# NicholasMilef/UUO-Mocap

Measured on AMD Instinct MI355X. Metric: mocap frames/sec fitted (300-frame seq, 50 markers), higher is better.
Workload: dtype f32

## Files before the change

uuo_mocap_amd/_lib.py:

```python
from __future__ import annotations

import ctypes
import os
import re
from ctypes import POINTER, c_char_p, c_float, c_int, c_int32, c_void_p

_HERE = os.path.dirname(os.path.abspath(__file__))
LIB_PATH = os.path.join(_HERE, "libuuo_hip.so")
HEADER_PATH = os.path.join(os.path.dirname(_HERE), "include", "uuo_hip.h")

UUO_STAGE_CHAMFER, UUO_STAGE_MARKER, UUO_STAGE_PART = 0, 1, 2


ABI_VERSION = 3


class UuoProblem(ctypes.Structure):
    _fields_ = [
        ("stage", c_int32), ("F", c_int32), ("M", c_int32),
        ("d_markers", c_void_p), ("d_o_pose", c_void_p), ("d_o_betas", c_void_p), ("d_root", c_void_p),
        ("d_assign", c_void_p), ("d_subset", c_void_p), ("n_subset", c_int32),
        ("w_data", c_float), ("w_pose", c_float), ("w_betas", c_float), ("marker_distance", c_float),
        ("pose_cache_id", ctypes.c_uint64),
        ("w_soft", c_float), ("soft_tau", c_float),
# ... 12 lines not shown
    _fields_ = [
        ("n_iter", c_int32), ("n_eval", c_int32), ("first_loss", c_float), ("final_loss", c_float),
        ("stop_reason", c_int32), ("device_ms", c_float),
    ]


class UuoReprojectionProblem(ctypes.Structure):
    _fields_ = [
        ("F", c_int32), ("M", c_int32), ("V", c_int32), ("J", c_int32),
        ("d_markers", c_void_p), ("d_joints0", c_void_p), ("d_verts0", c_void_p), ("d_kp_target", c_void_p),
        ("d_mask", c_void_p), ("focal", c_float * 2), ("center", c_float * 2),
        ("w_reprojection", c_float), ("w_chamfer", c_float),
    ]


EVAL_CALLBACK = ctypes.CFUNCTYPE(None, c_void_p, c_int, c_float, c_void_p)
GATHER_FN = ctypes.CFUNCTYPE(c_int, c_void_p, POINTER(ctypes.c_double), c_int, POINTER(ctypes.c_double))


class UuoShared(ctypes.Structure):
    _fields_ = [("gather", GATHER_FN), ("user", c_void_p), ("rank", c_int32), ("world", c_int32)]


_SIGNATURES = {
    "uuo_last_error": (c_char_p, []),
    "uuo_abi_version": (c_int, []),
    "uuo_model_create": (c_int, [c_void_p] * 7 + [c_int, POINTER(c_void_p)]),
    "uuo_model_destroy": (c_int, [c_void_p]),
    "uuo_model_num_verts": (c_int, [c_void_p]),
    "uuo_smpl_forward": (c_int, [c_void_p, c_void_p, c_int, c_void_p, c_void_p, c_int, c_void_p, c_void_p,
                                 c_void_p, c_void_p]),
    "uuo_smpl_backward": (c_int, [c_void_p, c_void_p, c_int, c_void_p, c_void_p, c_int, c_void_p, c_void_p, c_void_p,
                                  c_void_p, c_void_p, c_void_p, c_void_p, c_void_p, c_void_p]),
    "uuo_nn_argmin": (c_int, [c_void_p, c_int, c_int, c_int, c_void_p, c_void_p, c_void_p, c_int, c_void_p,
                              c_void_p, c_void_p]),
    "uuo_rigid_distance_std": (c_int, [c_void_p, c_int, c_int, c_void_p, c_void_p]),
    "uuo_assign_mean_argmin": (c_int, [c_void_p, c_int, c_int, c_int, c_void_p, c_void_p, c_void_p, c_void_p,
                                       c_void_p]),
    "uuo_soft_nn_forward": (c_int, [c_void_p, c_int, c_int, c_int, c_void_p, c_void_p, c_float, c_void_p, c_void_p,
                                    c_void_p, c_void_p]),
    "uuo_soft_nn_backward": (c_int, [c_void_p, c_int, c_int, c_int, c_void_p, c_void_p, c_float, c_void_p, c_void_p,
                                     c_void_p, c_void_p, c_void_p]),
    "uuo_copy_to_host": (c_int, [c_void_p, c_void_p, c_void_p, c_int]),
    "uuo_mesh_closest_points": (c_int, [c_void_p, c_int, c_int, c_int, c_int, c_void_p, c_void_p, c_void_p, c_void_p,
                                        c_void_p, c_void_p, c_void_p]),
    "uuo_fit_create": (c_int, [c_void_p, c_int, c_int, POINTER(c_void_p)]),
    "uuo_fit_destroy": (c_int, [c_void_p]),
    "uuo_problem_num_params": (c_int, [POINTER(UuoProblem)]),
    "uuo_closure_eval": (c_int, [c_void_p, c_void_p, POINTER(UuoProblem), c_void_p, c_void_p, c_void_p, c_void_p]),
    "uuo_lbfgs_solve": (c_int, [c_void_p, c_void_p, POINTER(UuoProblem), c_void_p, POINTER(UuoLbfgsOptions),
                                POINTER(UuoLbfgsStats), c_void_p, c_void_p]),
    "uuo_lbfgs_solve_shared": (c_int, [c_void_p, c_void_p, POINTER(UuoProblem), c_void_p, POINTER(UuoLbfgsOptions),
                                       POINTER(UuoLbfgsStats), POINTER(UuoShared), c_void_p, c_void_p]),
    "uuo_time_closure": (c_int, [c_void_p, c_void_p, POINTER(UuoProblem), c_void_p, c_int, c_int,
                                 POINTER(c_float)]),
    "uuo_lbfgs_minimize": (c_int, [c_void_p, c_int, c_void_p, POINTER(UuoLbfgsOptions), POINTER(UuoLbfgsStats), c_void_p,
                                   c_void_p, c_void_p, c_void_p]),
    "uuo_reprojection_create": (c_int, [POINTER(UuoReprojectionProblem), POINTER(c_void_p)]),
    "uuo_reprojection_destroy": (c_int, [c_void_p]),
    "uuo_reprojection_num_params": (c_int, [POINTER(UuoReprojectionProblem)]),
    "uuo_reprojection_eval": (c_int, [c_void_p, c_void_p, c_void_p, c_void_p, c_void_p, c_void_p, c_void_p]),
    "uuo_reprojection_solve": (c_int, [c_void_p, c_void_p, c_void_p, POINTER(UuoLbfgsOptions), POINTER(UuoLbfgsStats),
                                       c_void_p, c_void_p, c_void_p, c_void_p]),
    "uuo_set_wait_policy": (c_int, [c_int, c_int]),
    "uuo_mailbox_open": (c_int, [c_char_p, c_int32, c_int32, ctypes.c_double, POINTER(c_void_p)]),
    "uuo_mailbox_close": (c_int, [c_void_p]),
    "uuo_mailbox_gather": (c_int, [c_void_p, c_void_p, c_int, c_void_p]),
    "uuo_mailbox_stats": (c_int, [c_void_p, POINTER(ctypes.c_ulonglong), POINTER(ctypes.c_ulonglong)]),
    "uuo_copy_device": (c_int, [c_void_p, c_void_p, c_void_p, ctypes.c_size_t]),
    "uuo_batch_create": (c_int, [c_void_p, c_int, c_int, c_int, c_int, POINTER(c_void_p)]),
    "uuo_batch_destroy": (c_int, [c_void_p]),
    "uuo_batch_solve": (c_int, [c_void_p, c_void_p, POINTER(UuoProblem), POINTER(c_void_p), c_int,
                                POINTER(UuoLbfgsOptions), POINTER(UuoLbfgsStats)]),
    "uuo_batch_part_scores": (c_int, [c_void_p, c_void_p, POINTER(UuoProblem), POINTER(c_void_p), c_int,
                                      POINTER(c_float)]),
}
LIB_DEBUG_PATH = os.path.join(_HERE, "libuuo_hip_debug.so")
_DEBUG_SIGNATURES = {
    "uuo_lbfgs_selftest": (c_int, [c_void_p, c_int, c_int, c_void_p, POINTER(UuoLbfgsOptions),
                                   POINTER(UuoLbfgsStats), c_void_p, c_void_p]),
    "uuo_debug_fit_buffers": (c_int, [c_void_p, c_void_p, c_void_p]),
    "uuo_debug_nn_flags": (c_int, [c_void_p, c_void_p]),
    "uuo_debug_skin16_check": (c_int, [c_void_p, c_int]),
    "uuo_debug_small_coeffs": (c_int, [c_int, c_int, c_int, c_void_p]),
    "uuo_debug_time_small": (c_int, [c_int, c_int, c_int, POINTER(c_float)]),
    "uuo_debug_index_map": (c_int, [c_int, c_int, c_int, c_void_p]),
    "uuo_debug_staging_script": (c_int, [c_void_p, c_int, ctypes.c_longlong, c_void_p]),
}

CLOSURE_FN = ctypes.CFUNCTYPE(c_int, c_void_p, c_void_p, c_void_p, c_void_p, c_void_p)

_lib = None
_lib_debug = None


def header_symbols():
    text = open(HEADER_PATH).read()
    text = re.sub(r"/\*.*?\*/", "", text, flags=re.S)
    names = re.findall(r"\b(uuo_[a-z0-9_]+)\s*\(", text)
    return sorted(set(n for n in names if n != "uuo_eval_callback_t"))


def load():
    global _lib
    if _lib is not None:
        return _lib
    if not os.path.isfile(LIB_PATH):
        raise RuntimeError(
            "libuuo_hip.so is missing (%s): run `python __graft_entry__.py` to build the HIP extension. "
            "There is no CPU fallback for the fitted path." % LIB_PATH)
    lib = ctypes.CDLL(LIB_PATH)
    for name in header_symbols():
        if not hasattr(lib, name):
            raise RuntimeError("libuuo_hip.so does not export %s declared in include/uuo_hip.h" % name)
    for name, (res, args) in _SIGNATURES.items():
        fn = getattr(lib, name)
        fn.restype = res
        fn.argtypes = args
    if lib.uuo_abi_version() != ABI_VERSION:
        raise RuntimeError("libuuo_hip.so has ABI version %d, this package binds version %d: rebuild it "
                           "(python __graft_entry__.py)" % (lib.uuo_abi_version(), ABI_VERSION))
    _lib = lib
    return lib


def load_debug():
    global _lib_debug
    if _lib_debug is not None:
        return _lib_debug
    if not os.path.isfile(LIB_DEBUG_PATH):
        raise RuntimeError("libuuo_hip_debug.so is missing (%s): run `python __graft_entry__.py`" % LIB_DEBUG_PATH)
    lib = ctypes.CDLL(LIB_DEBUG_PATH)
    for name, (res, args) in list(_SIGNATURES.items()) + list(_DEBUG_SIGNATURES.items()):
        fn = getattr(lib, name)
        fn.restype = res
        fn.argtypes = args
    _lib_debug = lib
    return lib


def check(rc: int, what: str = ""):
    if rc != 0:
        msg = load().uuo_last_error()
        raise RuntimeError("%s failed (%d): %s" % (what or "libuuo_hip call", rc, msg.decode() if msg else ""))
```

uuo_mocap_amd/csrc/smpl_kernels.hip:

```cpp
#include <cstdlib>

#include "frame_math.h"


__device__ __forceinline__ void pose_prep_body(const UuoPoseSrc& src, const UuoTree* __restrict__ tree, int F,
                                               float* __restrict__ pfaT, float* __restrict__ A,
                                               float* __restrict__ jposed, float* __restrict__ frames,
                                               const float* __restrict__ ST = nullptr, const int* __restrict__ Wi = nullptr,
                                               const float* __restrict__ Ww = nullptr, int V = 0,
                                               const int32_t* __restrict__ subset = nullptr, int ns = 0,
                                               float* __restrict__ sb_out = nullptr, _Float16* __restrict__ pfa16 = nullptr) {
  __builtin_amdgcn_s_setprio(3);
  __shared__ FrameLds L;
  const int f = blockIdx.x;
  const int l = threadIdx.x;
  frame_forward(src, tree, f, L);
  if (frames) {
    constexpr int NW = sizeof(FrameLds) / 4;
    const float* src_l = reinterpret_cast<const float*>(&L);
    for (int i = l; i < NW; i += 64) frames[(size_t)f * NW + i] = src_l[i];
  }
  const int ft = f / UUO_FT, i = f % UUO_FT;
  float* tile = pfaT + (size_t)ft * UUO_KP * UUO_FT;
  _Float16* tile16 = pfa16 ? pfa16 + (size_t)ft * UUO_KP * UUO_FT * 2 : nullptr;
// ... 566 lines not shown
    ra[0] = pa[0];
#pragma unroll
    for (int g = 0; g < SKIN_GROUPS; ++g) {
      const int st = g % SK2_RING;
      const float4 av = ra[g & 1];
      const int part = g % 3;
      const int k_aread = (g < 12 && part == 2) ? 11 : 10;
#pragma unroll
      for (int k = 0; k < 12; ++k) {
        const int ks = k / 3, c = k - 3 * ks;
        const float a = (ks == 0) ? av.x : (ks == 1) ? av.y : (ks == 2) ? av.z : av.w;
        if (VAR & 4) {
          asm volatile("" ::"v"(a), "v"(rbuf[c][st][ks]));
        } else if (c == 0) {
          acc0 = __builtin_amdgcn_mfma_f32_16x16x4f32(a, rbuf[0][st][ks], acc0, 0, 0, 0);
        } else if (c == 1) {
          acc1 = __builtin_amdgcn_mfma_f32_16x16x4f32(a, rbuf[1][st][ks], acc1, 0, 0, 0);
        } else {
          acc2 = __builtin_amdgcn_mfma_f32_16x16x4f32(a, rbuf[2][st][ks], acc2, 0, 0, 0);
        }
        if (!(VAR & 1) && g < 12) sk2_slice<BBOX, VPOUT>(g, k, E, ww, q0, q1, q2, sTb, sTrb, v12, n24, rv, rb, rvp);
        if (k == k_aread && g + 1 < SKIN_GROUPS) ra[(g + 1) & 1] = pa[(g + 1) * 64];
        if (g == 2 && k == 11) {
          const int t_n = __builtin_amdgcn_readfirstlane(claimed);
          more = t_n < tb1;
          t_nxt = more ? t_n : t_cur;
          SK2_DECODE(nxt, t_nxt);
          pbn = (unsigned)nxt.u * (SKIN_GROUPS * 1024u);
        }
        if (g == 11 && k == 10) {
          wi = __builtin_bit_cast(int4, __builtin_amdgcn_raw_buffer_load_b128(rwi, j16, cur.u * 256, 0));
          ww = __builtin_bit_cast(float4, __builtin_amdgcn_raw_buffer_load_b128(rww, j16, cur.u * 256, 0));
          tn0 = __builtin_bit_cast(float, __builtin_amdgcn_raw_buffer_load_b32(rvt, j4, nxt.u * 64, 0));
          tn1 = __builtin_bit_cast(float, __builtin_amdgcn_raw_buffer_load_b32(rvt, j4, VP * 4 + nxt.u * 64, 0));
          tn2 = __builtin_bit_cast(float, __builtin_amdgcn_raw_buffer_load_b32(rvt, j4, VP * 8 + nxt.u * 64, 0));
        }
        __builtin_amdgcn_sched_barrier(0);
      }
      if (!(VAR & 2)) {
        const unsigned ub = (g + SK2_RING < SKIN_GROUPS) ? pb : pbn;
        const int gg = (g + SK2_RING) % SKIN_GROUPS;
        rbuf[0][st] = SK2_LDB(0, ub, gg);
        rbuf[1][st] = SK2_LDB(1, ub, gg);
        rbuf[2][st] = SK2_LDB(2, ub, gg);
      }
      __builtin_amdgcn_sched_barrier(0);
    }
    if (VAR & 8) {
      typedef unsigned u32x2 __attribute__((ext_vector_type(2)));
      const unsigned long long c = __builtin_readcyclecounter();
      const u32x2 cv = {(unsigned)c, (unsigned)(c >> 32)};
      const unsigned so = (unsigned)(((blockIdx.x * SKIN_WAVES + wave) * 16 + 2 + (nunits_done < 8 ? nunits_done : 7)) * 8);
      __builtin_amdgcn_raw_buffer_store_b64(cv, rst, so | (lane == 0 ? 0u : 0x80000000u), 0, 0);
    }
    ++nunits_done;
    q0 = acc0; q1 = acc1; q2 = acc2;
    prv = cur; cur = nxt; pb = pbn; t_cur = t_nxt;
    sk2_unit_addresses(E, prv, wi, kq, j, V, v12, n24);
  }
#undef SK2_LDB
#undef SK2_DECODE
#pragma unroll
  for (int g = 0; g < 12; ++g) {
#pragma unroll
    for (int k = 0; k < 12; ++k) sk2_slice<BBOX, VPOUT>(g, k, E, ww, q0, q1, q2, sTb, sTrb, v12, n24, rv, rb, rvp);
  }
  if ((VAR & 8) && lane == 0) {
    unsigned long long* o = g_sk2_stamps + (size_t)(blockIdx.x * SKIN_WAVES + wave) * 16;
    o[0] = stamp0; o[1] = stamp1;
    o[10] = __builtin_readcyclecounter();
    o[11] = (unsigned long long)nunits_done;
    o[12] = stampS;
  }
}

typedef _Float16 f16x8 __attribute__((ext_vector_type(8)));
#define SK3_STEPS (SKIN_GROUPS / 2)
#define SK3_NMFMA (SK3_STEPS * 9)
#define SK3_NSLICE 144

#ifndef SK3_WAVES
#define SK3_WAVES 4
#endif
#ifndef SK3_LDS_PAD
#define SK3_LDS_PAD 44288
#endif
template <bool BBOX>
__global__ __launch_bounds__(SK3_WAVES * 64) __attribute__((amdgpu_waves_per_eu(1, 1))) void k_skin3(
    const float4* __restrict__ P16v, const float* __restrict__ vt3, const int* __restrict__ Wi, const float* __restrict__ Ww,
    const float4* __restrict__ pfa16, const float* __restrict__ A, const float* __restrict__ trans, float* __restrict__ verts,
    float* __restrict__ bbox, int F, int V, int VP, int nFT, float inv_scale) {
  __shared__ float4 sA[2 * UUO_KP * UUO_FT / 4];
  __shared__ f32x4 sT[2 * UUO_FT * UUO_NUM_JOINTS * 3];
  __shared__ float4 sTr[2 * UUO_FT];
  __shared__ int sQ[64];
  const int tid = threadIdx.x;
  const int wave = __builtin_amdgcn_readfirstlane(tid >> 6), lane = tid & 63;
  const int j = lane & 15, kq = lane >> 4;
  const int nunits = VP / 16;
  const int nur = (V + 15) / 16;
  const int xcd = blockIdx.x & 7, pos = blockIdx.x >> 3;
  const int ntot = nFT * nur;
  const int xlo = (int)(((unsigned)ntot * (unsigned)xcd) >> 3), xhi = (int)(((unsigned)ntot * (unsigned)(xcd + 1)) >> 3);
  const int tb0 = xlo + (((xhi - xlo) * pos) >> SK2_NPOS_LOG2), tb1 = xlo + (((xhi - xlo) * (pos + 1)) >> SK2_NPOS_LOG2);
  if (tb1 <= tb0) return;
  int xa = 0;
  while (xa < 7 && nFT * (((xa + 1) * nur) >> 3) <= tb0) ++xa;
  const int ua0 = (xa * nur) >> 3, ub0 = ((xa + 1) * nur) >> 3;
  const int nua = ub0 - ua0;
  const int Sa = nFT * ua0, Sb = nFT * ub0;
  const int ftA = (tb0 - Sa) / nua;
  const int g1 = Sa + ftA * nua;
  const int g2 = (g1 + nua < Sb) ? g1 + nua : Sb;
  const int ftB = (tb1 - 1 < Sb) ? ftA + 1 : 0;
  const int nslots = (tb1 > g2) ? 2 : 1;

  const __amdgpu_buffer_rsrc_t rv = __builtin_amdgcn_make_buffer_rsrc(verts, 0, F * V * 12, 0x00020000);
  const __amdgpu_buffer_rsrc_t rb = __builtin_amdgcn_make_buffer_rsrc(bbox, 0, BBOX ? F * nur * 24 : 0, 0x00020000);
  const unsigned cplane = (unsigned)nunits * SKIN_GROUPS * 1024u;
  const __amdgpu_buffer_rsrc_t rp =
      __builtin_amdgcn_make_buffer_rsrc(const_cast<float4*>(P16v), 0, (int)(3u * cplane), 0x00020000);
  const __amdgpu_buffer_rsrc_t rwi = __builtin_amdgcn_make_buffer_rsrc(const_cast<int*>(Wi), 0, VP * 16, 0x00020000);
  const __amdgpu_buffer_rsrc_t rww = __builtin_amdgcn_make_buffer_rsrc(const_cast<float*>(Ww), 0, VP * 16, 0x00020000);
  const __amdgpu_buffer_rsrc_t rvt = __builtin_amdgcn_make_buffer_rsrc(const_cast<float*>(vt3), 0, VP * 12, 0x00020000);
  const unsigned lane16 = lane * 16, j16 = j * 16, j4 = j * 4;
#define SK3_LDB(c, ubase, g) \
  __builtin_bit_cast(f32x4, __builtin_amdgcn_raw_buffer_load_b128(rp, lane16, (ubase) + (c)*cplane + (g)*1024u, 0))
#define SK3_DECODE(U, t_)                                                        \
  {                                                                              \
    const bool s1_ = (t_) < g2;                                                  \
    const int base_ = s1_ ? g1 : ((t_) < Sb ? g2 : Sb);                          \
    (U).u = (((t_) < Sb) ? ua0 : ub0) + (t_)-base_;                              \
    (U).i0 = (s1_ ? ftA : ftB) * UUO_FT;                                         \
    (U).slot = s1_ ? 0 : 1;                                                      \
  }

  constexpr int NA = UUO_KP * UUO_FT / 4, NT = UUO_FT * UUO_NUM_JOINTS * 3;
  constexpr int PER = (2 * (NA + NT) + SK3_WAVES * 64 - 1) / (SK3_WAVES * 64);
  float4 tmp[PER];
  float4 trv = make_float4(0.f, 0.f, 0.f, 0.f);
  {
    const float4* gA0 = pfa16 + (size_t)ftA * NA;
    const float4* gA1 = pfa16 + (size_t)ftB * NA;
    const float4* gT0 = reinterpret_cast<const float4*>(A + (size_t)ftA * UUO_FT * UUO_NUM_JOINTS * 12);
    const float4* gT1 = reinterpret_cast<const float4*>(A + (size_t)ftB * UUO_FT * UUO_NUM_JOINTS * 12);
#pragma unroll
    for (int r = 0; r < PER; ++r) {
      const int i = tid + r * SK3_WAVES * 64;
      tmp[r] = make_float4(0.f, 0.f, 0.f, 0.f);
      if (i < NA) tmp[r] = gA0[i];
      else if (i < 2 * NA) { if (nslots > 1) tmp[r] = gA1[i - NA]; }
      else if (i < 2 * NA + NT) tmp[r] = gT0[i - 2 * NA];
      else if (i < 2 * NA + 2 * NT) { if (nslots > 1) tmp[r] = gT1[i - 2 * NA - NT]; }
    }
    if (tid < 2 * UUO_FT) {
      const int f = ((tid < UUO_FT) ? ftA : ftB) * UUO_FT + (tid & (UUO_FT - 1));
      if (trans && f < F && (tid < UUO_FT || nslots > 1))
        trv = make_float4(trans[(size_t)f * 3], trans[(size_t)f * 3 + 1], trans[(size_t)f * 3 + 2], 0.f);
    }
  }

  int t_cur = tb0 + wave;
  const bool active = t_cur < tb1;
  if (!active) t_cur = tb0;
  Sk2Unit cur, prv, nxt;
  SK3_DECODE(cur, t_cur);
  prv.u = cur.u; prv.i0 = F; prv.slot = 0;
  nxt = cur;
  unsigned pb = (unsigned)cur.u * (SKIN_GROUPS * 1024u);
  f32x4 rbuf[3][SK2_RING];
#pragma unroll
  for (int s = 0; s < SK2_RING; ++s) {
    rbuf[0][s] = SK3_LDB(0, pb, s);
    rbuf[1][s] = SK3_LDB(1, pb, s);
    rbuf[2][s] = SK3_LDB(2, pb, s);
  }

  if (tid < 64) sQ[tid] = (tid == 0) ? tb0 + SK3_WAVES : 0;
#pragma unroll
  for (int r = 0; r < PER; ++r) {
    const int i = tid + r * SK3_WAVES * 64;
    if (i < 2 * NA) sA[i] = tmp[r];
    else if (i < 2 * (NA + NT)) sT[i - 2 * NA] = __builtin_bit_cast(f32x4, tmp[r]);
  }
  if (tid < 2 * UUO_FT) sTr[tid] = trv;
  __syncthreads();
  if (!active) return;

  int4 wi = make_int4(0, 0, 0, 0);
  float4 ww = make_float4(0.f, 0.f, 0.f, 0.f);
  f32x4 q0 = {0.f, 0.f, 0.f, 0.f}, q1 = q0, q2 = q0;
  Sk2Epi E;
  const char* sTb = reinterpret_cast<const char*>(sT);
  const char* sTrb = reinterpret_cast<const char*>(sTr);
  const unsigned v12 = (unsigned)V * 12u, n24 = (unsigned)nur * 24u;
  sk2_unit_addresses(E, prv, wi, kq, j, V, v12, n24);
  bool more = true;

  while (more) {
    const int claimed = __hip_atomic_fetch_add(&sQ[lane], lane == 0 ? 1 : 0, __ATOMIC_RELAXED, __HIP_MEMORY_SCOPE_WORKGROUP);
    unsigned pbn = pb;
    int t_nxt = t_cur;
    const float tn0 = __builtin_bit_cast(float, __builtin_amdgcn_raw_buffer_load_b32(rvt, j4, cur.u * 64, 0));
    const float tn1 = __builtin_bit_cast(float, __builtin_amdgcn_raw_buffer_load_b32(rvt, j4, VP * 4 + cur.u * 64, 0));
    const float tn2 = __builtin_bit_cast(float, __builtin_amdgcn_raw_buffer_load_b32(rvt, j4, VP * 8 + cur.u * 64, 0));
    const int4 wi_n = __builtin_bit_cast(int4, __builtin_amdgcn_raw_buffer_load_b128(rwi, j16, cur.u * 256, 0));
    const float4 ww_n = __builtin_bit_cast(float4, __builtin_amdgcn_raw_buffer_load_b128(rww, j16, cur.u * 256, 0));
    const float4* pa = sA + cur.slot * (UUO_KP * UUO_FT / 4) + lane;
    f32x4 am0 = {0.f, 0.f, 0.f, 0.f}, am1 = am0, am2 = am0;
    f32x4 as0 = am0, as1 = am0, as2 = am0;
    float4 ah[2], al[2];
    ah[0] = pa[0];
    al[0] = pa[64];
#ifdef SK3_NO_MFMA
#define SK3_MFMA(acc, a_, b_) asm volatile("" : "+v"(acc) : "v"(a_), "v"(b_))
#else
#define SK3_MFMA(acc, a_, b_) asm volatile("v_mfma_f32_16x16x32_f16 %0, %1, %2, %0" : "+v"(acc) : "v"(a_), "v"(b_))
#endif
#define SK3_STEP(ST)                                                         \
    {                                                                        \
      constexpr int st = ST;                                                 \
      constexpr int rh = (2 * st) % SK2_RING, rl = (2 * st + 1) % SK2_RING; \
      const f16x8 a_hi = __builtin_bit_cast(f16x8, ah[st & 1]), a_lo = __builtin_bit_cast(f16x8, al[st & 1]); \
_Pragma("unroll") \
      for (int q = 0; q < 9; ++q) { \
        const int term = q / 3, c = q - 3 * term; \
        const f16x8 b_hi = __builtin_bit_cast(f16x8, rbuf[c][rh]), b_lo = __builtin_bit_cast(f16x8, rbuf[c][rl]); \
        const f16x8 ax = (term == 2) ? a_lo : a_hi, bx = (term == 1) ? b_lo : b_hi; \
        if (term == 0) { \
          if (c == 0) SK3_MFMA(am0, ax, bx); \
          else if (c == 1) SK3_MFMA(am1, ax, bx); \
          else SK3_MFMA(am2, ax, bx); \
        } else { \
          if (c == 0) SK3_MFMA(as0, ax, bx); \
          else if (c == 1) SK3_MFMA(as1, ax, bx); \
          else SK3_MFMA(as2, ax, bx); \
        } \
        const int mslot = st * 9 + q; \
        const int n0 = (mslot * SK3_NSLICE) / SK3_NMFMA, n1 = ((mslot + 1) * SK3_NSLICE) / SK3_NMFMA; \
_Pragma("unroll") \
        for (int i = 0; i < 3; ++i) { \
          const int n = n0 + i; \
          if (n < n1) sk2_slice<BBOX, false, true>(n / 12, n % 12, E, ww, q0, q1, q2, sTb, sTrb, v12, n24, rv, rb, rv); \
        } \
        if (q == 5 && st + 1 < SK3_STEPS) { \
          ah[(st + 1) & 1] = pa[(2 * (st + 1)) * 64]; \
          al[(st + 1) & 1] = pa[(2 * (st + 1) + 1) * 64]; \
        } \
        if (st == 2 && q == 4) { \
          const int t_n = __builtin_amdgcn_readfirstlane(claimed); \
          more = t_n < tb1; \
          t_nxt = more ? t_n : t_cur; \
          SK3_DECODE(nxt, t_nxt); \
          pbn = (unsigned)nxt.u * (SKIN_GROUPS * 1024u); \
        } \
        __builtin_amdgcn_sched_barrier(0); \
      } \
      { \
        constexpr int gh = 2 * st + SK2_RING, gl = 2 * st + 1 + SK2_RING; \
        const unsigned ubh = (gh < SKIN_GROUPS) ? pb : pbn, ubl = (gl < SKIN_GROUPS) ? pb : pbn; \
        rbuf[0][rh] = SK3_LDB(0, ubh, gh % SKIN_GROUPS); \
        rbuf[1][rh] = SK3_LDB(1, ubh, gh % SKIN_GROUPS); \
        rbuf[2][rh] = SK3_LDB(2, ubh, gh % SKIN_GROUPS); \
        rbuf[0][rl] = SK3_LDB(0, ubl, gl % SKIN_GROUPS); \
        rbuf[1][rl] = SK3_LDB(1, ubl, gl % SKIN_GROUPS); \
        rbuf[2][rl] = SK3_LDB(2, ubl, gl % SKIN_GROUPS); \
      } \
      __builtin_amdgcn_sched_barrier(0); \
    }
    SK3_STEP(0) SK3_STEP(1) SK3_STEP(2) SK3_STEP(3) SK3_STEP(4) SK3_STEP(5) SK3_STEP(6)
#undef SK3_STEP
#undef SK3_MFMA
    asm volatile("s_nop 7\n\ts_nop 3");
    __builtin_amdgcn_sched_barrier(0);
    q0 = (am0 + as0) * inv_scale + tn0;
    q1 = (am1 + as1) * inv_scale + tn1;
    q2 = (am2 + as2) * inv_scale + tn2;
    wi = wi_n;
    ww = ww_n;
    prv = cur; cur = nxt; pb = pbn; t_cur = t_nxt;
    sk2_unit_addresses(E, prv, wi, kq, j, V, v12, n24);
  }
#undef SK3_LDB
#undef SK3_DECODE
#pragma unroll
  for (int g = 0; g < 12; ++g) {
#pragma unroll
    for (int k = 0; k < 12; ++k) sk2_slice<BBOX, false, true>(g, k, E, ww, q0, q1, q2, sTb, sTrb, v12, n24, rv, rb, rv);
  }
}

static bool sk2_fits(int nFT, int nur, int npos) {
  if (nur < 8) return false;
  const int ntot = nFT * nur;
  for (int x = 0; x < 8; ++x) {
    const int xlo = (int)(((long)ntot * x) >> 3), xhi = (int)(((long)ntot * (x + 1)) >> 3);
    for (int pos = 0; pos < npos; ++pos) {
      const int tb0 = xlo + (((xhi - xlo) * pos) >> SK2_NPOS_LOG2), tb1 = xlo + (((xhi - xlo) * (pos + 1)) >> SK2_NPOS_LOG2);
      if (tb1 <= tb0) continue;
      int xa = 0;
      while (xa < 7 && nFT * (((xa + 1) * nur) >> 3) <= tb0) ++xa;
      const int ua0 = (xa * nur) >> 3, ub0 = ((xa + 1) * nur) >> 3, nua = ub0 - ua0;
      const int Sa = nFT * ua0, Sb = nFT * ub0;
      const int ftA = (tb0 - Sa) / nua;
      const int g1 = Sa + ftA * nua;
      const int g2 = (g1 + nua < Sb) ? g1 + nua : Sb;
      const bool seg2 = tb1 > g2 && g2 < Sb;
      const bool seg3 = tb1 > Sb;
      if (seg2 && seg3) return false;
      if (seg2 && tb1 > g2 + nua) return false;
      if (seg3 && (xa >= 7 || tb1 - Sb > (((xa + 2) * nur) >> 3) - ub0)) return false;
    }
  }
  return true;
}

static int uuo_launch_skin_v1(const uuo_model* m, hipStream_t s, int F, const float* pfaT, const float* A,
                              const float* trans, float* verts, float* bbox);

struct SkinCallArgs {
  UuoGridHdr h;
  const uuo_model* m;
  int F;
  const float* pfaT;
  const float* A;
  const float* trans;
  float* verts;
  float* bbox;
  const void* pfa16;
};

int uuo_launch_skin(const uuo_model* m, hipStream_t s, int F, const float* pfaT, const float* A, const float* trans,
                    float* verts, float* bbox, float* vp_out) {
  UUO_REQUIRE(!vp_out || (bbox && !uuo_recorder), "uuo_launch_skin: v_posed output goes with the unit boxes, outside lock-step batches");
  {
    SkinCallArgs c{{1, 1}, m, F, pfaT, A, trans, verts, bbox, nullptr};
    if (uuo_record(UUO_OP_SKIN, 1, 1, c)) return 0;
  }
  static const int force_v1 = UUO_ENV_INT("UUO_SKIN_V1", 0);
  const int nur = (m->V + 15) / 16;
  const int npos = 1 << SK2_NPOS_LOG2;
  if (force_v1 || (size_t)SK2_MAX_FT * UUO_FT * m->V * 12 >= 0x7FFFFFF0u) {
    UUO_REQUIRE(!vp_out, "uuo_launch_skin: v_posed output needs the k_skin2 path");
    return uuo_launch_skin_v1(m, s, F, pfaT, A, trans, verts, bbox);
  }
  const int nFT_all = (F + UUO_FT - 1) / UUO_FT;
  for (int ft0 = 0; ft0 < nFT_all; ft0 += SK2_MAX_FT) {
    const int nFT = (nFT_all - ft0 < SK2_MAX_FT) ? nFT_all - ft0 : SK2_MAX_FT;
    const int f0 = ft0 * UUO_FT;
    const int Fl = (F - f0 < nFT * UUO_FT) ? F - f0 : nFT * UUO_FT;
    if (!sk2_fits(nFT, nur, npos)) {
      UUO_REQUIRE(!vp_out, "uuo_launch_skin: v_posed output needs the k_skin2 path");
      return uuo_launch_skin_v1(m, s, F, pfaT, A, trans, verts, bbox);
    }
    const float* pf = pfaT + (size_t)ft0 * UUO_KP * UUO_FT;
    const float* pA = A + (size_t)f0 * UUO_NUM_JOINTS * 12;
    const float* pt = trans ? trans + (size_t)f0 * 3 : nullptr;
    float* pv = verts + (size_t)f0 * m->V * 3;
    static const int var2 = UUO_ENV_INT("UUO_SK2_VAR", 0);
#define SK2_LAUNCH(BB, VAR)                                                                             \
  hipLaunchKernelGGL((k_skin2<BB, VAR>), dim3(8 * npos), dim3(SKIN_WAVES * 64), 0, s,                   \
                     reinterpret_cast<const float4*>(m->P3), m->vt3, m->Wi, m->Ww, pf, pA, pt, pv,      \
                     (BB) ? bbox + (size_t)f0 * nur * 6 : (float*)nullptr, Fl, m->V, m->VP, nFT, (float*)nullptr)
    if (!bbox) SK2_LAUNCH(false, 0);
    else if (vp_out)
      hipLaunchKernelGGL((k_skin2<true, 0, true>), dim3(8 * npos), dim3(SKIN_WAVES * 64), 0, s,
                         reinterpret_cast<const float4*>(m->P3), m->vt3, m->Wi, m->Ww, pf, pA, pt, pv,
                         bbox + (size_t)f0 * nur * 6, Fl, m->V, m->VP, nFT, vp_out + (size_t)f0 * m->V * 3);
#ifdef UUO_DEBUG_HOOKS
    else if (var2 == 1) SK2_LAUNCH(true, 1);
    else if (var2 == 2) SK2_LAUNCH(true, 2);
    else if (var2 == 4) SK2_LAUNCH(true, 4);
    else if (var2 == 3) SK2_LAUNCH(true, 3);
    else if (var2 == 5) SK2_LAUNCH(true, 5);
    else if (var2 == 6) SK2_LAUNCH(true, 6);
    else if (var2 == 7) SK2_LAUNCH(true, 7);
    else if (var2 == 16) SK2_LAUNCH(false, 0);
    else if (var2 == 8) SK2_LAUNCH(true, 8);
    else if (var2 == 9) SK2_LAUNCH(true, 9);
    else if (var2 == 10) SK2_LAUNCH(true, 10);
    else if (var2 == 11) SK2_LAUNCH(true, 11);
    else if (var2 == 12) SK2_LAUNCH(true, 12);
    else if (var2 == 24) SK2_LAUNCH(false, 8);
#endif
    else SK2_LAUNCH(true, 0);
    (void)var2;
#undef SK2_LAUNCH
  }
  UUO_HIP_CHECK(hipGetLastError());
  return 0;
}

#ifdef UUO_DEBUG_HOOKS
extern "C" int uuo_debug_skin_stamps(unsigned long long* h_out) {
  UUO_HIP_CHECK(hipMemcpyFromSymbol(h_out, HIP_SYMBOL(g_sk2_stamps), sizeof(unsigned long long) * 2048 * 16));
  return 0;
}
#endif

int uuo_launch_skin16(const uuo_model* m, hipStream_t s, int F, const void* pfa16, const float* A, const float* trans, float* verts,
                      float* bbox) {
  UUO_REQUIRE(m->P16 && pfa16 && bbox, "uuo_launch_skin16: needs the fp16 tables and the unit boxes");
  static const hipError_t lds_attr =
      hipFuncSetAttribute(reinterpret_cast<const void*>(&k_skin3<true>), hipFuncAttributeMaxDynamicSharedMemorySize, SK3_LDS_PAD);
  UUO_HIP_CHECK(lds_attr);
  const int nur = (m->V + 15) / 16;
  const int npos = 1 << SK2_NPOS_LOG2;
  if ((size_t)SK2_MAX_FT * UUO_FT * m->V * 12 >= 0x7FFFFFF0u) return -22;
  const int nFT_all = (F + UUO_FT - 1) / UUO_FT;
  for (int ft0 = 0; ft0 < nFT_all; ft0 += SK2_MAX_FT) {
    const int nFT = (nFT_all - ft0 < SK2_MAX_FT) ? nFT_all - ft0 : SK2_MAX_FT;
    if (!sk2_fits(nFT, nur, npos)) return -22;
  }
  {
    SkinCallArgs c{{1, 1}, m, F, nullptr, A, trans, verts, bbox, pfa16};
    if (uuo_record(UUO_OP_SKIN, 1, 1, c)) return 0;
  }
  for (int ft0 = 0; ft0 < nFT_all; ft0 += SK2_MAX_FT) {
    const int nFT = (nFT_all - ft0 < SK2_MAX_FT) ? nFT_all - ft0 : SK2_MAX_FT;
    const int f0 = ft0 * UUO_FT;
    const int Fl = (F - f0 < nFT * UUO_FT) ? F - f0 : nFT * UUO_FT;
    hipLaunchKernelGGL((k_skin3<true>), dim3(8 * npos), dim3(SK3_WAVES * 64), SK3_LDS_PAD, s, reinterpret_cast<const float4*>(m->P16), m->vt3,
                       m->Wi, m->Ww, reinterpret_cast<const float4*>(pfa16) + (size_t)ft0 * (UUO_KP * UUO_FT / 4),
                       A + (size_t)f0 * UUO_NUM_JOINTS * 12, trans ? trans + (size_t)f0 * 3 : (const float*)nullptr,
                       verts + (size_t)f0 * m->V * 3, bbox + (size_t)f0 * nur * 6, Fl, m->V, m->VP, nFT, m->skin16_inv);
  }
  UUO_HIP_CHECK(hipGetLastError());
  return 0;
}

static int uuo_launch_skin_v1(const uuo_model* m, hipStream_t s, int F, const float* pfaT, const float* A,
                              const float* trans, float* verts, float* bbox) {
  const int nFT = (F + UUO_FT - 1) / UUO_FT;
  const int nunits = m->VP / 16;
  static const int slots = UUO_ENV_INT("UUO_SKIN_SLOTS", 256);
  int nVB = slots / nFT;
  const int maxVB = (nunits + SKIN_WAVES - 1) / SKIN_WAVES;
  if (nVB > maxVB) nVB = maxVB;
  if (nVB < 1) nVB = 1;
  const int nblocks = nFT * nVB;
  static const int variant = UUO_ENV_INT("UUO_SKIN_VARIANT", 0);
#define SKIN_LAUNCH(VAR)                                                                                     \
  hipLaunchKernelGGL((k_skin<VAR>), dim3(nblocks), dim3(SKIN_WAVES * 64), 0, s, m->P3, m->vt3, m->Wi, m->Ww, \
                     pfaT, A, trans, verts, bbox, F, m->V, m->VP, nFT, nVB, nblocks)
#ifdef UUO_DEBUG_HOOKS
  if (variant == 1) SKIN_LAUNCH(1);
  else if (variant == 2) SKIN_LAUNCH(2);
  else if (variant == 3) SKIN_LAUNCH(3);
  else if (variant == 4) SKIN_LAUNCH(4);
  else if (variant == 5) SKIN_LAUNCH(5);
  else
#endif
    SKIN_LAUNCH(0);
  (void)variant;
#undef SKIN_LAUNCH
  UUO_HIP_CHECK(hipGetLastError());
  return 0;
}

#define SKC_FB 10
__device__ __forceinline__ void skin_cached_body(int F, int V, int ns, const int32_t* __restrict__ subset,
                                                 const float* __restrict__ C, const float* __restrict__ ST,
                                                 const int* __restrict__ Wi, const float* __restrict__ Ww,
                                                 const float* __restrict__ A, const float* __restrict__ betas,
                                                 const float* __restrict__ trans, float* __restrict__ verts,
                                                 float* __restrict__ bbox) {
  __shared__ float sA[SKC_FB * UUO_NUM_JOINTS * 12];
  __shared__ float sTr[SKC_FB * 3];
  const int f0 = blockIdx.y * SKC_FB, nf = min(SKC_FB, F - f0);
  for (int i = threadIdx.x; i < nf * UUO_NUM_JOINTS * 12; i += 256) sA[i] = A[(size_t)f0 * UUO_NUM_JOINTS * 12 + i];
  if (threadIdx.x < nf * 3) sTr[threadIdx.x] = trans ? trans[(size_t)f0 * 3 + threadIdx.x] : 0.f;
  __syncthreads();
  const int i = blockIdx.x * 256 + threadIdx.x;
  const bool compact = bbox != nullptr;
  if (!compact && i >= ns) return;
  if (compact && (i & ~15) >= ns) return;
  const bool mine = i < ns;
  const int ic = mine ? i : ns - 1;
  const int v = subset ? subset[ic] : ic;
  if ((unsigned)v >= (unsigned)V) {
    if (!compact) return;
  }
  const int vs = ((unsigned)v < (unsigned)V) ? v : 0;
  float sb[3] = {0.f, 0.f, 0.f};
#pragma unroll
  for (int c = 0; c < 3; ++c)
#pragma unroll
    for (int l = 0; l < 10; ++l) sb[c] = fmaf(ST[(size_t)vs * 30 + c * 10 + l], betas[l], sb[c]);
  const int4 wi = *reinterpret_cast<const int4*>(Wi + (size_t)vs * 4);
  const float4 ww = *reinterpret_cast<const float4*>(Ww + (size_t)vs * 4);
  const int wj[4] = {wi.x, wi.y, wi.z, wi.w};
  const float wv[4] = {ww.x, ww.y, ww.z, ww.w};
  const int nuc = (ns + 15) >> 4;
  float cx[SKC_FB], cy[SKC_FB], cz[SKC_FB];
#pragma unroll
  for (int q = 0; q < SKC_FB; ++q) {
    const float* pc = C + ((size_t)(f0 + (q < nf ? q : nf - 1)) * V + vs) * 3;
    cx[q] = pc[0]; cy[q] = pc[1]; cz[q] = pc[2];
  }
#pragma unroll
  for (int q = 0; q < SKC_FB; ++q) {
    if (q >= nf) continue;
    const float px = cx[q] + sb[0], py = cy[q] + sb[1], pz = cz[q] + sb[2];
    float T[12];
#pragma unroll
    for (int e = 0; e < 12; ++e) T[e] = 0.f;
#pragma unroll
    for (int n = 0; n < 4; ++n) {
      const float* a = sA + (q * UUO_NUM_JOINTS + (wj[n] < 0 ? 0 : wj[n])) * 12;
      const float w = (wj[n] < 0) ? 0.f : wv[n];
// ... 160 lines not shown
```

Measured before the change: 1452.

## Restructure fp16 skinning kernel to keep basis in AGPRs across frame tiles

Replaces the skin3 kernel with a version where each wave owns a quad of vertex units and streams frame tiles through a three-slot LDS ring. The fp16 basis for the current units is loaded once into accumulation registers and reused across all frame tiles, then prefetched for the next quad during the MFMA steps. The first MFMA per accumulator now uses a zero source instead of a zeroed register. The grid becomes a fixed 256 blocks with a linear split of work, and the old kernel is kept as a debug reference with a bitwise comparator. The cost is higher register and LDS pressure and more complex scheduling.

```diff
diff --git a/uuo_mocap_amd/_lib.py b/uuo_mocap_amd/_lib.py
--- a/uuo_mocap_amd/_lib.py
+++ b/uuo_mocap_amd/_lib.py
@@ -118,6 +118,7 @@
     "uuo_debug_fit_buffers": (c_int, [c_void_p, c_void_p, c_void_p]),
     "uuo_debug_nn_flags": (c_int, [c_void_p, c_void_p]),
     "uuo_debug_skin16_check": (c_int, [c_void_p, c_int]),
+    "uuo_debug_skin16_ref_check": (c_int, [c_void_p, c_int]),
     "uuo_debug_small_coeffs": (c_int, [c_int, c_int, c_int, c_void_p]),
     "uuo_debug_time_small": (c_int, [c_int, c_int, c_int, POINTER(c_float)]),
     "uuo_debug_index_map": (c_int, [c_int, c_int, c_int, c_void_p]),
diff --git a/uuo_mocap_amd/csrc/smpl_kernels.hip b/uuo_mocap_amd/csrc/smpl_kernels.hip
--- a/uuo_mocap_amd/csrc/smpl_kernels.hip
+++ b/uuo_mocap_amd/csrc/smpl_kernels.hip
@@ -672,11 +672,11 @@
 #ifndef SK3_WAVES
 #define SK3_WAVES 4
 #endif
-#ifndef SK3_LDS_PAD
-#define SK3_LDS_PAD 44288
-#endif
+#define SK3_LDS_TOTAL 110592
+#ifdef UUO_DEBUG_HOOKS
+#define SK3_REF_LDS_PAD (SK3_LDS_TOTAL - 66304)
 template <bool BBOX>
-__global__ __launch_bounds__(SK3_WAVES * 64) __attribute__((amdgpu_waves_per_eu(1, 1))) void k_skin3(
+__global__ __launch_bounds__(SK3_WAVES * 64) __attribute__((amdgpu_waves_per_eu(1, 1))) void k_skin3_ref(
     const float4* __restrict__ P16v, const float* __restrict__ vt3, const int* __restrict__ Wi, const float* __restrict__ Ww,
     const float4* __restrict__ pfa16, const float* __restrict__ A, const float* __restrict__ trans, float* __restrict__ verts,
     float* __restrict__ bbox, int F, int V, int VP, int nFT, float inv_scale) {
@@ -805,7 +805,13 @@
 #ifdef SK3_NO_MFMA
 #define SK3_MFMA(acc, a_, b_) asm volatile("" : "+v"(acc) : "v"(a_), "v"(b_))
 #else
-#define SK3_MFMA(acc, a_, b_) asm volatile("v_mfma_f32_16x16x32_f16 %0, %1, %2, %0" : "+v"(acc) : "v"(a_), "v"(b_))
+#define SK3_MFMA(acc, a_, b_)                                                                                        \
+  do {                                                                                                               \
+    if (st == 0 && q < 6)                                                                                            \
+      asm volatile("v_mfma_f32_16x16x32_f16 %0, %1, %2, 0" : "=&v"(acc) : "v"(a_), "v"(b_));                        \
+    else                                                                                                             \
+      asm volatile("v_mfma_f32_16x16x32_f16 %0, %1, %2, %0" : "+v"(acc) : "v"(a_), "v"(b_));                        \
+  } while (0)
 #endif
 #define SK3_STEP(ST)                                                         \
     {                                                                        \
@@ -879,6 +885,220 @@
     for (int k = 0; k < 12; ++k) sk2_slice<BBOX, false, true>(g, k, E, ww, q0, q1, q2, sTb, sTrb, v12, n24, rv, rb, rv);
   }
 }
+#endif
+
+#define SK3_NBLK 256
+#define SK3_SLOTS 3
+#define SK3_TILE_BYTES (UUO_KP * UUO_FT * 4 + UUO_FT * UUO_NUM_JOINTS * 48 + UUO_FT * 16)
+#define SK3_LDS_PAD (SK3_LDS_TOTAL - SK3_SLOTS * SK3_TILE_BYTES)
+
+__host__ __device__ __forceinline__ void sk3_run(int ntot, int b, int& t0, int& t1) {
+  const unsigned lin = (unsigned)(b & 7) * (SK3_NBLK / 8) + (unsigned)(b >> 3);
+  t0 = (int)(((unsigned)ntot * lin) / SK3_NBLK);
+  t1 = (int)(((unsigned)ntot * (lin + 1)) / SK3_NBLK);
+}
+
+template <bool BBOX>
+__global__ __launch_bounds__(SK3_WAVES * 64) __attribute__((amdgpu_waves_per_eu(1, 1))) void k_skin3(
+    const float4* __restrict__ P16v, const float* __restrict__ vt3, const int* __restrict__ Wi, const float* __restrict__ Ww,
+    const float4* __restrict__ pfa16, const float* __restrict__ A, const float* __restrict__ trans, float* __restrict__ verts,
+    float* __restrict__ bbox, int F, int V, int VP, int nFT, float inv_scale) {
+  constexpr int NA = UUO_KP * UUO_FT / 4, NT = UUO_FT * UUO_NUM_JOINTS * 3;
+  constexpr int PER = (NA + NT) / (SK3_WAVES * 64);
+  static_assert(PER * SK3_WAVES * 64 == NA + NT && NA % 64 == 0, "a tile is 8 float4 per thread, each wave's either A or T");
+  static_assert(SK3_SLOTS * SK3_TILE_BYTES + SK3_LDS_PAD == SK3_LDS_TOTAL && SK3_LDS_PAD >= 0, "LDS footprint");
+  __shared__ float4 sA[SK3_SLOTS * NA];
+  __shared__ f32x4 sT[SK3_SLOTS * NT];
+  __shared__ float4 sTr[SK3_SLOTS * UUO_FT];
+  const int tid = threadIdx.x;
+  const int wave = __builtin_amdgcn_readfirstlane(tid >> 6), lane = tid & 63;
+  const int j = lane & 15, kq = lane >> 4;
+  const int nunits = VP / 16;
+  const int nur = (V + 15) / 16;
+  const int ntot = ((nur + 3) >> 2) * nFT;
+  int tb0, tb1;
+  sk3_run(ntot, blockIdx.x, tb0, tb1);
+  if (tb1 <= tb0) return;
+
+  const __amdgpu_buffer_rsrc_t rv = __builtin_amdgcn_make_buffer_rsrc(verts, 0, F * V * 12, 0x00020000);
+  const __amdgpu_buffer_rsrc_t rb = __builtin_amdgcn_make_buffer_rsrc(bbox, 0, BBOX ? F * nur * 24 : 0, 0x00020000);
+  const unsigned cplane = (unsigned)nunits * SKIN_GROUPS * 1024u;
+  const __amdgpu_buffer_rsrc_t rp =
+      __builtin_amdgcn_make_buffer_rsrc(const_cast<float4*>(P16v), 0, (int)(3u * cplane), 0x00020000);
+  const __amdgpu_buffer_rsrc_t rwi = __builtin_amdgcn_make_buffer_rsrc(const_cast<int*>(Wi), 0, VP * 16, 0x00020000);
+  const __amdgpu_buffer_rsrc_t rww = __builtin_amdgcn_make_buffer_rsrc(const_cast<float*>(Ww), 0, VP * 16, 0x00020000);
+  const __amdgpu_buffer_rsrc_t rvt = __builtin_amdgcn_make_buffer_rsrc(const_cast<float*>(vt3), 0, VP * 12, 0x00020000);
+  const unsigned lane16 = lane * 16, j16 = j * 16, j4 = j * 4;
+  float4 tmp[PER];
+  float4 trv;
+#define SK3_STAGE_LOAD(ft_)                                                                                 \
+  {                                                                                                         \
+    const float4* gA_ = pfa16 + (size_t)(ft_) * NA;                                                         \
+    const float4* gT_ = reinterpret_cast<const float4*>(A + (size_t)(ft_) * UUO_FT * UUO_NUM_JOINTS * 12); \
+    _Pragma("unroll") for (int r = 0; r < PER; ++r) {                                                       \
+      const int i = tid + r * SK3_WAVES * 64;                                                               \
+      tmp[r] = *((i < NA) ? gA_ + i : gT_ + (i - NA));                                                      \
+    }                                                                                                       \
+    trv = make_float4(0.f, 0.f, 0.f, 0.f);                                                                  \
+    const int f_ = (ft_) * UUO_FT + tid;                                                                    \
+    if (tid < UUO_FT && trans && f_ < F)                                                                    \
+      trv = make_float4(trans[(size_t)f_ * 3], trans[(size_t)f_ * 3 + 1], trans[(size_t)f_ * 3 + 2], 0.f);  \
+  }
+#define SK3_STAGE_STORE(slot_)                                                       \
+  {                                                                                  \
+    _Pragma("unroll") for (int r = 0; r < PER; ++r) {                                \
+      const int i = tid + r * SK3_WAVES * 64;                                        \
+      if (i < NA) sA[(slot_) * NA + i] = tmp[r];                                     \
+      else sT[(slot_) * NT + i - NA] = __builtin_bit_cast(f32x4, tmp[r]);          \
+    }                                                                                \
+    if (tid < UUO_FT) sTr[(slot_) * UUO_FT + tid] = trv;                             \
+  }
+#define SK3_BARRIER()                                                      \
+  {                                                                        \
+    __builtin_amdgcn_sched_barrier(0);                                     \
+    asm volatile("s_waitcnt lgkmcnt(0)\n\ts_barrier" ::: "memory");        \
+    __builtin_amdgcn_sched_barrier(0);                                     \
+  }
+
+  f32x4 bas[3][SKIN_GROUPS];
+#define SK3_LOAD_STEP(st_, ubase)                                                                                         \
+  {                                                                                                                        \
+    const unsigned o_ = (ubase) + (2 * (st_)) * 1024u;                                                                     \
+    asm volatile("s_nop 4\n\t"                                                                                             \
+                 "buffer_load_dwordx4 %0, %6, %7, %8 offen\n\t"                                                           \
+                 "buffer_load_dwordx4 %1, %6, %7, %9 offen\n\t"                                                           \
+                 "buffer_load_dwordx4 %2, %6, %7, %10 offen\n\t"                                                          \
+                 "buffer_load_dwordx4 %3, %6, %7, %8 offen offset:1024\n\t"                                               \
+                 "buffer_load_dwordx4 %4, %6, %7, %9 offen offset:1024\n\t"                                               \
+                 "buffer_load_dwordx4 %5, %6, %7, %10 offen offset:1024"                                                  \
+                 : "=a"(bas[0][2 * (st_)]), "=a"(bas[1][2 * (st_)]), "=a"(bas[2][2 * (st_)]), "=a"(bas[0][2 * (st_) + 1]), \
+                   "=a"(bas[1][2 * (st_) + 1]), "=a"(bas[2][2 * (st_) + 1])                                               \
+                 : "v"(lane16), "s"(rp), "s"(o_), "s"(o_ + cplane), "s"(o_ + 2 * cplane));                               \
+  }
+  int quad = tb0 / nFT, ft = tb0 - quad * nFT;
+  SK3_STAGE_LOAD(ft);
+  {
+    const unsigned pb = (unsigned)(4 * quad + wave) * (SKIN_GROUPS * 1024u);
+    SK3_LOAD_STEP(0, pb) SK3_LOAD_STEP(1, pb) SK3_LOAD_STEP(2, pb) SK3_LOAD_STEP(3, pb)
+    SK3_LOAD_STEP(4, pb) SK3_LOAD_STEP(5, pb) SK3_LOAD_STEP(6, pb)
+  }
+  SK3_STAGE_STORE(0);
+  SK3_BARRIER();
+  bool basis_in_flight = true;
+
+  int4 wi = make_int4(0, 0, 0, 0);
+  float4 ww = make_float4(0.f, 0.f, 0.f, 0.f);
+  f32x4 q0 = {0.f, 0.f, 0.f, 0.f}, q1 = q0, q2 = q0;
+  Sk2Epi E;
+  const char* sTb = reinterpret_cast<const char*>(sT);
+  const char* sTrb = reinterpret_cast<const char*>(sTr);
+  const unsigned v12 = (unsigned)V * 12u, n24 = (unsigned)nur * 24u;
+  Sk2Unit cur, prv;
+  prv.u = 4 * quad + wave; prv.i0 = F; prv.slot = 0;
+  sk2_unit_addresses(E, prv, wi, kq, j, V, v12, n24);
+  int slot = 0;
+
+  for (int t = tb0; t < tb1; ++t) {
+    cur.u = 4 * quad + wave; cur.i0 = ft * UUO_FT; cur.slot = slot;
+    const bool more = t + 1 < tb1;
+    const int ftn = (ft + 1 < nFT) ? ft + 1 : 0;
+    const int quadn = (ft + 1 < nFT) ? quad : quad + 1;
+    const bool reload = more && quadn != quad;
+    const unsigned pbn = (unsigned)(4 * quadn + wave) * (SKIN_GROUPS * 1024u);
+    const int slotn = (slot == SK3_SLOTS - 1) ? 0 : slot + 1;
+    if (basis_in_flight) {
+      __builtin_amdgcn_sched_barrier(0);
+      asm volatile("s_waitcnt vmcnt(0)" ::: "memory");
+      __builtin_amdgcn_sched_barrier(0);
+    }
+    basis_in_flight = reload;
+    if (more) SK3_STAGE_LOAD(ftn);
+    const float tn0 = __builtin_bit_cast(float, __builtin_amdgcn_raw_buffer_load_b32(rvt, j4, cur.u * 64, 0));
+    const float tn1 = __builtin_bit_cast(float, __builtin_amdgcn_raw_buffer_load_b32(rvt, j4, VP * 4 + cur.u * 64, 0));
+    const float tn2 = __builtin_bit_cast(float, __builtin_amdgcn_raw_buffer_load_b32(rvt, j4, VP * 8 + cur.u * 64, 0));
+    const int4 wi_n = __builtin_bit_cast(int4, __builtin_amdgcn_raw_buffer_load_b128(rwi, j16, cur.u * 256, 0));
+    const float4 ww_n = __builtin_bit_cast(float4, __builtin_amdgcn_raw_buffer_load_b128(rww, j16, cur.u * 256, 0));
+    const float4* pa = sA + cur.slot * NA + lane;
+    f32x4 am0 = {0.f, 0.f, 0.f, 0.f}, am1 = am0, am2 = am0;
+    f32x4 as0 = am0, as1 = am0, as2 = am0;
+    float4 ah[2], al[2];
+    ah[0] = pa[0];
+    al[0] = pa[64];
+#define SK3_PIN(st_)                                                                                                        \
+  asm volatile("s_nop 4" : "+a"(bas[0][2 * (st_)]), "+a"(bas[1][2 * (st_)]), "+a"(bas[2][2 * (st_)]),                    \
+               "+a"(bas[0][2 * (st_) + 1]), "+a"(bas[1][2 * (st_) + 1]), "+a"(bas[2][2 * (st_) + 1]));                  \
+  __builtin_amdgcn_sched_barrier(0)
+#define SK3_MFMA(acc, a_, b_)                                                                                        \
+  do {                                                                                                               \
+    if (st == 0 && q < 6)                                                                                            \
+      asm volatile("v_mfma_f32_16x16x32_f16 %0, %1, %2, 0" : "=&v"(acc) : "v"(a_), "a"(b_));                        \
+    else                                                                                                             \
+      asm volatile("v_mfma_f32_16x16x32_f16 %0, %1, %2, %0" : "+v"(acc) : "v"(a_), "a"(b_));                        \
+  } while (0)
+#define SK3_STEP(ST)                                                         \
+    {                                                                        \
+      constexpr int st = ST;                                                 \
+      const f16x8 a_hi = __builtin_bit_cast(f16x8, ah[st & 1]), a_lo = __builtin_bit_cast(f16x8, al[st & 1]); \
+      SK3_PIN(st); \
+_Pragma("unroll") \
+      for (int q = 0; q < 9; ++q) { \
+        const int term = q / 3, c = q - 3 * term; \
+        const f16x8 b_hi = __builtin_bit_cast(f16x8, bas[c][2 * st]), b_lo = __builtin_bit_cast(f16x8, bas[c][2 * st + 1]); \
+        const f16x8 ax = (term == 2) ? a_lo : a_hi, bx = (term == 1) ? b_lo : b_hi; \
+        if (term == 0) { \
+          if (c == 0) SK3_MFMA(am0, ax, bx); \
+          else if (c == 1) SK3_MFMA(am1, ax, bx); \
+          else SK3_MFMA(am2, ax, bx); \
+        } else { \
+          if (c == 0) SK3_MFMA(as0, ax, bx); \
+          else if (c == 1) SK3_MFMA(as1, ax, bx); \
+          else SK3_MFMA(as2, ax, bx); \
+        } \
+        const int mslot = st * 9 + q; \
+        const int n0 = (mslot * SK3_NSLICE) / SK3_NMFMA, n1 = ((mslot + 1) * SK3_NSLICE) / SK3_NMFMA; \
+_Pragma("unroll") \
+        for (int i = 0; i < 3; ++i) { \
+          const int n = n0 + i; \
+          if (n < n1) sk2_slice<BBOX, false, true>(n / 12, n % 12, E, ww, q0, q1, q2, sTb, sTrb, v12, n24, rv, rb, rv); \
+        } \
+        if (q == 5 && st + 1 < SK3_STEPS) { \
+          ah[(st + 1) & 1] = pa[(2 * (st + 1)) * 64]; \
+          al[(st + 1) & 1] = pa[(2 * (st + 1) + 1) * 64]; \
+        } \
+        __builtin_amdgcn_sched_barrier(0); \
+      } \
+      if (reload) SK3_LOAD_STEP(st, pbn) \
+      __builtin_amdgcn_sched_barrier(0); \
+    }
+    SK3_STEP(0) SK3_STEP(1) SK3_STEP(2) SK3_STEP(3) SK3_STEP(4) SK3_STEP(5) SK3_STEP(6)
+#undef SK3_STEP
+#undef SK3_MFMA
+#undef SK3_PIN
+    asm volatile("s_nop 7\n\ts_nop 3");
+    __builtin_amdgcn_sched_barrier(0);
+    q0 = (am0 + as0) * inv_scale + tn0;
+    q1 = (am1 + as1) * inv_scale + tn1;
+    q2 = (am2 + as2) * inv_scale + tn2;
+    wi = wi_n;
+    ww = ww_n;
+    if (more) {
+      SK3_STAGE_STORE(slotn);
+      SK3_BARRIER();
+    }
+    prv = cur; quad = quadn; ft = ftn; slot = slotn;
+    sk2_unit_addresses(E, prv, wi, kq, j, V, v12, n24);
+    if (prv.u >= nur) E.bo |= 0x80000000u;
+  }
+#undef SK3_LOAD_STEP
+#undef SK3_STAGE_LOAD
+#undef SK3_STAGE_STORE
+#undef SK3_BARRIER
+#pragma unroll
+  for (int g = 0; g < 12; ++g) {
+#pragma unroll
+    for (int k = 0; k < 12; ++k) sk2_slice<BBOX, false, true>(g, k, E, ww, q0, q1, q2, sTb, sTrb, v12, n24, rv, rb, rv);
+  }
+}
 
 static bool sk2_fits(int nFT, int nur, int npos) {
   if (nur < 8) return false;
@@ -988,6 +1208,79 @@
 }
 #endif
 
+#ifdef UUO_DEBUG_HOOKS
+static int g_sk3_ref_on = 0;
+static float* g_sk3_ref_buf = nullptr;
+static size_t g_sk3_ref_cap = 0;
+__device__ unsigned long long g_sk3_ref_count[24];
+__global__ __launch_bounds__(256) void k_skin16_bitwise(const unsigned* __restrict__ a, const unsigned* __restrict__ b, size_t n,
+                                                        const unsigned* __restrict__ ba, const unsigned* __restrict__ bb, size_t nb,
+                                                        int V) {
+  const size_t i0 = (size_t)blockIdx.x * 256 + threadIdx.x, stride = (size_t)gridDim.x * 256;
+  unsigned bad = 0, badb = 0;
+  for (size_t i = i0; i < n; i += stride) {
+    if (a[i] != b[i]) {
+      ++bad;
+      atomicAdd(&g_sk3_ref_count[4 + (i / ((size_t)V * 3)) % 16], 1ull);
+      atomicAdd(&g_sk3_ref_count[20 + i % 3], 1ull);
+    }
+  }
+  for (size_t i = i0; i < nb; i += stride) badb += (ba[i] != bb[i]) ? 1u : 0u;
+  if (bad) atomicAdd(&g_sk3_ref_count[1], (unsigned long long)bad);
+  if (badb) atomicAdd(&g_sk3_ref_count[2], (unsigned long long)badb);
+  if (i0 == 0) atomicAdd(&g_sk3_ref_count[0], 1ull);
+}
+static int sk3_ref_compare(const uuo_model* m, hipStream_t s, int F, const void* pfa16, const float* A, const float* trans,
+                           const float* verts, const float* bbox) {
+  hipStreamCaptureStatus cs = hipStreamCaptureStatusNone;
+  UUO_HIP_CHECK(hipStreamIsCapturing(s, &cs));
+  if (cs != hipStreamCaptureStatusNone) return 0;
+  static const hipError_t lds_attr = hipFuncSetAttribute(reinterpret_cast<const void*>(&k_skin3_ref<true>),
+                                                         hipFuncAttributeMaxDynamicSharedMemorySize, SK3_REF_LDS_PAD);
+  UUO_HIP_CHECK(lds_attr);
+  const int nur = (m->V + 15) / 16;
+  const size_t nv = (size_t)F * m->V * 3, nb = (size_t)F * nur * 6;
+  if (g_sk3_ref_cap < nv + nb) {
+    UUO_HIP_CHECK(hipDeviceSynchronize());
+    if (g_sk3_ref_buf) UUO_HIP_CHECK(hipFree(g_sk3_ref_buf));
+    UUO_HIP_CHECK(hipMalloc((void**)&g_sk3_ref_buf, (nv + nb) * sizeof(float)));
+    g_sk3_ref_cap = nv + nb;
+  }
+  float* rverts = g_sk3_ref_buf;
+  float* rbox = g_sk3_ref_buf + nv;
+  UUO_HIP_CHECK(hipMemsetAsync(g_sk3_ref_buf, 0xff, (nv + nb) * sizeof(float), s));
+  const int nFT_all = (F + UUO_FT - 1) / UUO_FT;
+  for (int ft0 = 0; ft0 < nFT_all; ft0 += SK2_MAX_FT) {
+    const int nFT = (nFT_all - ft0 < SK2_MAX_FT) ? nFT_all - ft0 : SK2_MAX_FT;
+    if (!sk2_fits(nFT, nur, 1 << SK2_NPOS_LOG2)) return -22;
+    const int f0 = ft0 * UUO_FT;
+    const int Fl = (F - f0 < nFT * UUO_FT) ? F - f0 : nFT * UUO_FT;
+    hipLaunchKernelGGL((k_skin3_ref<true>), dim3(8 << SK2_NPOS_LOG2), dim3(SK3_WAVES * 64), SK3_REF_LDS_PAD, s,
+                       reinterpret_cast<const float4*>(m->P16), m->vt3, m->Wi, m->Ww,
+                       reinterpret_cast<const float4*>(pfa16) + (size_t)ft0 * (UUO_KP * UUO_FT / 4),
+                       A + (size_t)f0 * UUO_NUM_JOINTS * 12, trans ? trans + (size_t)f0 * 3 : (const float*)nullptr,
+                       rverts + (size_t)f0 * m->V * 3, rbox + (size_t)f0 * nur * 6, Fl, m->V, m->VP, nFT, m->skin16_inv);
+  }
+  hipLaunchKernelGGL(k_skin16_bitwise, dim3(512), dim3(256), 0, s, reinterpret_cast<const unsigned*>(verts),
+                     reinterpret_cast<const unsigned*>(rverts), nv, reinterpret_cast<const unsigned*>(bbox),
+                     reinterpret_cast<const unsigned*>(rbox), nb, m->V);
+  UUO_HIP_CHECK(hipGetLastError());
+  return 0;
+}
+extern "C" int uuo_debug_skin16_ref_check(unsigned long long* h_out, int mode) {
+  UUO_HIP_CHECK(hipDeviceSynchronize());
+  unsigned long long h[24] = {};
+  if (mode == 1) {
+    UUO_HIP_CHECK(hipMemcpyToSymbol(HIP_SYMBOL(g_sk3_ref_count), h, sizeof(h)));
+  } else {
+    UUO_HIP_CHECK(hipMemcpyFromSymbol(h, HIP_SYMBOL(g_sk3_ref_count), sizeof(h)));
+  }
+  if (h_out) for (int i = 0; i < (mode == 2 ? 24 : 3); ++i) h_out[i] = h[i];
+  g_sk3_ref_on = mode == 1;
+  return 0;
+}
+#endif
+
 int uuo_launch_skin16(const uuo_model* m, hipStream_t s, int F, const void* pfa16, const float* A, const float* trans, float* verts,
                       float* bbox) {
   UUO_REQUIRE(m->P16 && pfa16 && bbox, "uuo_launch_skin16: needs the fp16 tables and the unit boxes");
@@ -995,27 +1288,27 @@
       hipFuncSetAttribute(reinterpret_cast<const void*>(&k_skin3<true>), hipFuncAttributeMaxDynamicSharedMemorySize, SK3_LDS_PAD);
   UUO_HIP_CHECK(lds_attr);
   const int nur = (m->V + 15) / 16;
-  const int npos = 1 << SK2_NPOS_LOG2;
-  if ((size_t)SK2_MAX_FT * UUO_FT * m->V * 12 >= 0x7FFFFFF0u) return -22;
-  const int nFT_all = (F + UUO_FT - 1) / UUO_FT;
-  for (int ft0 = 0; ft0 < nFT_all; ft0 += SK2_MAX_FT) {
-    const int nFT = (nFT_all - ft0 < SK2_MAX_FT) ? nFT_all - ft0 : SK2_MAX_FT;
-    if (!sk2_fits(nFT, nur, npos)) return -22;
-  }
+  const size_t tile_bytes = (size_t)UUO_FT * m->V * 12;
+  const int max_ft = (int)((size_t)0x7FFFFFF0u / tile_bytes);
+  if (nur < 8 || max_ft < 1 || F < 1) return -22;
   {
     SkinCallArgs c{{1, 1}, m, F, nullptr, A, trans, verts, bbox, pfa16};
     if (uuo_record(UUO_OP_SKIN, 1, 1, c)) return 0;
   }
-  for (int ft0 = 0; ft0 < nFT_all; ft0 += SK2_MAX_FT) {
-    const int nFT = (nFT_all - ft0 < SK2_MAX_FT) ? nFT_all - ft0 : SK2_MAX_FT;
+  const int nFT_all = (F + UUO_FT - 1) / UUO_FT;
+  for (int ft0 = 0; ft0 < nFT_all; ft0 += max_ft) {
+    const int nFT = (nFT_all - ft0 < max_ft) ? nFT_all - ft0 : max_ft;
     const int f0 = ft0 * UUO_FT;
     const int Fl = (F - f0 < nFT * UUO_FT) ? F - f0 : nFT * UUO_FT;
-    hipLaunchKernelGGL((k_skin3<true>), dim3(8 * npos), dim3(SK3_WAVES * 64), SK3_LDS_PAD, s, reinterpret_cast<const float4*>(m->P16), m->vt3,
-                       m->Wi, m->Ww, reinterpret_cast<const float4*>(pfa16) + (size_t)ft0 * (UUO_KP * UUO_FT / 4),
+    hipLaunchKernelGGL((k_skin3<true>), dim3(SK3_NBLK), dim3(SK3_WAVES * 64), SK3_LDS_PAD, s, reinterpret_cast<const float4*>(m->P16),
+                       m->vt3, m->Wi, m->Ww, reinterpret_cast<const float4*>(pfa16) + (size_t)ft0 * (UUO_KP * UUO_FT / 4),
                        A + (size_t)f0 * UUO_NUM_JOINTS * 12, trans ? trans + (size_t)f0 * 3 : (const float*)nullptr,
                        verts + (size_t)f0 * m->V * 3, bbox + (size_t)f0 * nur * 6, Fl, m->V, m->VP, nFT, m->skin16_inv);
   }
   UUO_HIP_CHECK(hipGetLastError());
+#ifdef UUO_DEBUG_HOOKS
+  if (g_sk3_ref_on) return sk3_ref_compare(m, s, F, pfa16, A, trans, verts, bbox);
+#endif
   return 0;
 }
 
```

Result: no change. 1461, median of 6 (+0.6%).
